# WeeFav/Visual-Odometry-GPU

Measured on AMD Instinct MI355X. Metric: ORB detect+describe frames/sec (1241x376, 8 lvls), higher is better.
Workload: dtype u8; 1 GPU; KITTI-shaped 1241x376 u8, 8 levels s=1.2, 1000 features, FAST-9 t=20, NMS 3x3, Harris top-N, blur5 all levels, BRIEF-256; batch=1024 frames/step/GPU resident in HBM (stream A); distinct_resident_batches=2, fast_early_exit=True, pyramid_blur_fused=True, pyramid_top_rows_first=True, pipelined_batches=True

## Files before the change

### visual-odometry-gpu_amd/csrc/orbx_api.cpp

```cpp
#include <algorithm>
#include <array>
#include <cmath>
#include <cstdlib>
#include <cstring>
#include <new>

#include "orbx_host.h"

using namespace orbx_host;

namespace {
thread_local std::string g_create_error;
}

namespace orbx_host {

int fail(orbx_ctx* c, int status, const std::string& msg) {
  if (c)
    c->err = msg;
  else
    g_create_error = msg;
  return status;
}

// ... 169 lines not shown
}

int pyr_group_env() {
  static const int v = env_int("ORBX_PYR_GROUP", 32);
  return v;
}

int top_rows_env() {
  static const int v = std::max(env_int("ORBX_TOP_ROWS", 2), 0);
  return v;
}

int fast_impl_env() { return env_int("ORBX_FAST_IMPL", 4) == 3 ? 3 : 4; }

void first_split_env(orbx_ctx* c) {
  const char* e = getenv("ORBX_TOP_ROWS");
  e = e ? std::strchr(e, ':') : nullptr;
  while (e && *e == ':') {
    e++;
    if (!std::strncmp(e, "equal", 5)) {
      c->first_split = false;
    } else if (!std::strncmp(e, "trace", 5)) {
      c->split_trace = true;
    } else {
      for (int l = 0; l < ORBX_MAX_LEVELS; l++) {
        char* end = nullptr;
        const long v = std::strtol(e, &end, 10);
        if (end == e) break;
        c->cut_force[l] = (int)std::min<long>(std::max<long>(v, 0), 0xffff);
        e = end;
        if (*e != ',') break;
        e++;
      }
    }
    e = std::strchr(e, ':');
  }
}
int fast_unit_rows_max(const orbx_ctx* c) {
  return c->fast_impl == 4 ? ORBX_FAST_UNIT_ROWS_MAX : orbx_fast3_tile_h(c->p.nms_window / 2);
}

void make_taps(OrbxPlan& plan, std::vector<OrbxResizeTap>* taps) {
  taps->assign(taps_count(plan), OrbxResizeTap{0, 0, 0});
  for (int l = 1; l < plan.nlevels; l++) {
    const OrbxLevel& L = plan.L[l];
    const double scale_x = 1. / ((double)L.w / plan.w0), scale_y = 1. / ((double)L.h / plan.h0);
// ... 167 lines not shown
    int first[ORBX_MAX_LEVELS][2] = {};
    bool any = false;
    for (int l = 0; l < plan.nlevels; l++) {
      int a = c->cut_force[l] > 0 ? c->cut_force[l] : c->cut_pref[l];
      if (a <= 0 || c->bm_fast.tiles_y[l] < 2) continue;
      const int depth = 2 * c->bm_fast.tile_h[l], umax = fast_unit_rows_max(c);
      if (c->cut_force[l] > 0)
        a = std::max(std::max(1, depth - umax), std::min(a, std::min(umax, std::min(depth, plan.L[l].h) - 1)));
      first[l][0] = a;
      first[l][1] = depth - a;
      any = true;
    }
    if (any)
      (void)make_bandmap(plan, c->p.nms_window / 2, &c->bm_fast, &why, c->fast_impl == 4,
                         c->prefs_applied ? c->tile_h_pref : nullptr, first);
  }
  const bool grouped = pyr_group_env() > 0;
  const int top = top_rows_env();
  std::vector<OrbxTileDesc> t;
  blur_tiles_for_impl(c->blur_impl, plan, &t);
  if ((st = upload_tiles(c, T_BLUR, t, "blur tile table exceeds pool")) != ORBX_OK) return st;
  build_pyrblur_tiles(plan, ORBX_PYRBLUR_RH, &t, grouped);
  if ((st = upload_tiles(c, T_PYRBLUR, t, "strip table exceeds pool")) != ORBX_OK) return st;
  build_pyrblur_tiles(plan, ORBX_PYRBLUR_RH, &t, grouped, 1, &c->bm_fast, top);
  if ((st = upload_tiles(c, T_PYRBLUR_TOP, t, "strip table exceeds pool")) != ORBX_OK) return st;
  build_pyrblur_tiles(plan, ORBX_PYRBLUR_RH, &t, grouped, 2, &c->bm_fast, top);
  if ((st = upload_tiles(c, T_PYRBLUR_REST, t, "strip table exceeds pool")) != ORBX_OK) return st;
  c->top_levels = OrbxTopLevels{};
  for (int l = 0; l < plan.nlevels; l++)
    if (pyrblur_first_pass_rows(plan, c->bm_fast, l, top) < plan.L[l].h) {
      const int i = c->top_levels.n++;
      c->top_levels.stat_index[i] = l * ORBX_MAX_BANDS;
      c->top_levels.rows[i] = std::min(top, c->bm_fast.tiles_y[l]);
      c->top_levels.cap[i] = plan.L[l].cap;
    }
  build_pyrblur_tiles(plan, ORBX_PYRBLUR_RH_SMALL, &t);
  if ((st = upload_tiles(c, T_PYRBLUR_SMALL, t, "strip table exceeds pool")) != ORBX_OK) return st;
  build_frame_tiles(plan, ORBX_PYR2_TW, ORBX_PYR2_TH, true, &t);
  if ((st = upload_tiles(c, T_PYR2, t, "pyramid tile table exceeds pool")) != ORBX_OK) return st;
  build_fast_tiles(plan, c->bm_fast, 0, 1, &t);
  if ((st = upload_tiles(c, T_FAST, t, "FAST tile table exceeds pool")) != ORBX_OK) return st;
  c->plan_serial++;
  c->plan_w = w;
  c->plan_h = h;
  return ORBX_OK;
}

hipError_t launch_pyramid_auto(orbx_ctx* c, hipStream_t s, int n, const uint8_t* d_in, int in_stride,
                               size_t in_frame_stride) {
// ... 94 lines not shown
    const int dflt = orbx_fast3_tile_h(c->p.nms_window / 2), lh = c->plan.L[l].h;
    const int bal = (lh + (lh + dflt - 1) / dflt - 1) / ((lh + dflt - 1) / dflt);
    int hh = (rows + top - 1) / top;
    if (c->fast_impl == 4) {
      const int over = (hh + 2 * (c->p.nms_window / 2)) % 7;
      if ((over == 1 || over == 2) && top * (hh - over) >= (int)need + 3) hh -= over;
    }
    if (hh >= bal || lh <= top * hh) hh = 0;
    const int eff = hh ? hh : bal, cur = c->bm_fast.tile_h[l], asked = c->tile_h_pref[l] ? c->tile_h_pref[l] : bal;
    want[l] = ((eff > cur && (int)need > top * cur) || eff + 2 < std::min(cur, asked)) ? hh : c->tile_h_pref[l];
    if (eff > cur && (int)need > top * cur) grow = true;
    else if (eff + 2 < std::min(cur, asked)) change = true;
  }
  const bool heights_change = grow || change;
  const bool split = c->first_split && top == 2 && c->fast_impl == 4;
  const int R = c->p.nms_window / 2;
  int cut_want[ORBX_MAX_LEVELS] = {};
  bool cut_change = false;
  for (int l = 0; l < nl; l++) {
    uint32_t hist[ORBX_FILL_BUCKETS];
    uint64_t total = 0;
    for (int b = 0; b < ORBX_FILL_BUCKETS; b++) {
      hist[b] = c->fill_cur[l][b] + c->fill_prev[l][b];
      c->fill_prev[l][b] = c->fill_cur[l][b];
      c->fill_cur[l][b] = 0;
      total += hist[b];
    }
    if (!split || c->cut_force[l] > 0 || c->bm_fast.tiles_y[l] < 2) continue;
    const int dflt = orbx_fast3_tile_h(R), lh = c->plan.L[l].h;
    const int bal = (lh + (lh + dflt - 1) / dflt - 1) / ((lh + dflt - 1) / dflt);
    const int th_after = heights_change ? (want[l] ? want[l] : bal) : c->bm_fast.tile_h[l];
    const int depth = 2 * th_after;
    const int in_force = !heights_change && c->bm_fast.first_h[l][0] > 0 ? c->bm_fast.first_h[l][0] : 0;
    int cost_new = 0;
    const int cut_new = total && lh > depth ? choose_first_cut(hist, depth, R, ORBX_FAST_UNIT_ROWS_MAX, &cost_new) : 0;
    const int cost_now = first_pass_cost_milli(hist, depth, in_force ? in_force : depth / 2, R);
    if (!total || lh <= depth) cost_new = cost_now;
    const bool pays = cost_now - cost_new >= 1000, stopped = in_force && !cut_new && cost_now > cost_new;
    cut_want[l] = heights_change || pays || stopped ? cut_new : c->cut_pref[l];
    if (cut_want[l] != in_force && (pays || stopped)) cut_change = true;
    if (c->split_trace) {
      fprintf(stderr, "orbx split: batch %lld level %d need %u depth %d cut %d -> %d (%d -> %d milli-groups) fill rows:",
              c->batch_serial, l, c->need_prev[l], depth, in_force, cut_want[l], cost_now, cost_new);
      for (int b = 0; b < ORBX_FILL_BUCKETS; b++)
        if (hist[b]) fprintf(stderr, " %d:%u", ORBX_FILL_BUCKET_ROWS * (b + 1), hist[b]);
      fprintf(stderr, "\n");
// ... 77 lines not shown
                                 (int32_t*)(B.d + o.counts), (orbx_keypoint*)(B.d + o.lkp),
                                 (float*)(B.d + o.resp), (int32_t*)(B.d + o.level),
                                 (orbx_keypoint*)(B.d + o.kp), (uint32_t*)(B.d + o.kp16),
                                 (float*)(B.d + o.angle),
                                 (orbx_descriptor*)(B.d + o.desc), two_pass ? c->d_feedback : nullptr,
                                 two_pass ? const_cast<uint32_t*>(c->h_feedback) : nullptr, &hr));
  HIPCHK(c, mark(7, false));
  return ORBX_OK;
}

void drop_graph(orbx_ctx* c, int i) {
  if (c->g_exec[i]) (void)hipGraphExecDestroy(c->g_exec[i]);
  c->g_exec[i] = nullptr;
}

int run_batch(orbx_ctx* c, const uint8_t* d_frames, int n, int w, int h, int row_stride, size_t frame_stride,
              hipStream_t s, bool may_pipeline = false) {
  if (w != c->learn_w || h != c->learn_h) {
    c->learn_w = w;
    c->learn_h = h;
    for (int l = 0; l < ORBX_MAX_LEVELS; l++) c->need_cur[l] = c->need_prev[l] = 0, c->tile_h_pref[l] = c->cut_pref[l] = 0;
    std::memset(c->fill_cur, 0, sizeof(c->fill_cur));
    std::memset(c->fill_prev, 0, sizeof(c->fill_prev));
    for (int i = 2; i < ORBX_FEEDBACK_WORDS; i++) c->h_feedback[i] = 0;
    c->need_batches = 0;
    c->need_window = 2;
    c->retiles = 0;
  } else if (w == c->plan_w && h == c->plan_h) {
    bool any_pref = false;
    for (int l = 0; l < ORBX_MAX_LEVELS; l++) any_pref |= c->tile_h_pref[l] != 0 || c->cut_pref[l] != 0 || c->cut_force[l] != 0;
    if (adapt_tile_rows(c) || (any_pref && tile_prefs_apply(c) != c->prefs_applied)) c->plan_w = 0;
  }
  const bool lanes = may_pipeline && c->pipelined && s == c->stream && w == c->plan_w && h == c->plan_h;
  c->lane = lanes ? c->next_lane : 0;
  Lane& L = c->lanes[c->lane];
  if (lanes) {
    s = L.stream;
  } else {
    if (c->lanes[1].stream) HIPCHK(c, lanes_sync(c));
    if (c->last_stream && c->last_stream != s) HIPCHK(c, hipStreamSynchronize(c->last_stream));
  }
  int st = set_plan(c, w, h);
  if (st != ORBX_OK) return st;
  top_rows_update(c);
  const int blk = (c->blk + 1) % orbx_ctx::kBlocks;
  Block& B = c->blocks[blk];
// ... 443 lines not shown
  *total = (long long)c->bm_fast.band_begin[c->bm_fast.nbands] * n;
  *worked = fast_early_on(c) ? w : *total;
  return ORBX_OK;
}

int orbx_pyramid_pixel_counts(orbx_ctx* c, long long* produced, long long* total) {
  DeviceGuard _dg(c);
  if (!c || !produced || !total) return ORBX_ERR_INVALID_ARG;
  if (c->plan_w == 0 || last_block(c).n < 1) return fail(c, ORBX_ERR_INVALID_ARG, "run a batch first");
  const int n = last_block(c).n, top = top_rows_env();
  long long per_frame = 0;
  for (int l = 0; l < c->plan.nlevels; l++) per_frame += (long long)c->plan.L[l].w * c->plan.L[l].h;
  *total = per_frame * n;
  *produced = *total;
  if (!c->last_two_pass) return ORBX_OK;
  std::vector<unsigned long long> h((size_t)n * ORBX_FAST_STAT_WORDS);
  HIPCHK(c, hipStreamSynchronize(c->last_stream));
  HIPCHK(c, hipMemcpy(h.data(), cur_lane(c).d_row_stat, h.size() * 8, hipMemcpyDeviceToHost));
  long long done = 0;
  for (int f = 0; f < n; f++)
    for (int l = 0; l < c->plan.nlevels; l++) {
      const OrbxLevel& L = c->plan.L[l];
      const int first = pyrblur_first_pass_rows(c->plan, c->bm_fast, l, top);
      long long surv = 0;
      for (int b = 0; b < std::min(top, c->bm_fast.tiles_y[l]); b++)
        surv += (long long)(uint32_t)h[(size_t)f * ORBX_FAST_STAT_WORDS + (size_t)l * ORBX_MAX_BANDS + b];
      done += (long long)L.w * (first < L.h && surv >= L.cap ? first : L.h);
    }
  *produced = done;
  return ORBX_OK;
}

int orbx_enable_stage_timing(orbx_ctx* c, int enable) {
  DeviceGuard _dg(c);
  if (!c) return ORBX_ERR_INVALID_ARG;
  c->timing = enable < 0 || enable > 2 ? 1 : enable;
  return ORBX_OK;
}

int orbx_stage_times_history(orbx_ctx* c, int back, float* ms) {
  DeviceGuard _dg(c);
  if (!c || !ms) return ORBX_ERR_INVALID_ARG;
  if (back < 0 || back >= ORBX_EVENT_SETS || back >= c->ev_calls)
    return fail(c, ORBX_ERR_INVALID_ARG, "no timed batched call that far back");
  const long long call = c->ev_calls - 1 - back;
  const TimingSet& ts = c->evr[call % ORBX_EVENT_SETS];
  const hipEvent_t* evs = ts.ev;
  const int mode = ts.mode;
  std::memset(ms, 0, sizeof(float) * ORBX_NUM_STAGE_TIMES);
  if (mode == 1) {
// ... 257 lines not shown
```

### visual-odometry-gpu_amd/csrc/orbx_host.h

```cpp
#pragma once
#include <hip/hip_runtime.h>

#include <cmath>
#include <cstring>
#include <initializer_list>
#include <string>
#include <vector>

#include "orbx_internal.h"
#include "orbx_layout.h"

namespace orbx_host {

using namespace orbx_geom;
using namespace orbx_layout;

struct DevBuf {
  void* p = nullptr;
  size_t bytes = 0;
};
template <class T>
T* at(const DevBuf& b, size_t off) { return reinterpret_cast<T*>(static_cast<uint8_t*>(b.p) + off); }
inline void free_bufs(std::initializer_list<DevBuf*> bufs) {
  for (DevBuf* b : bufs)
// ... 274 lines not shown
  orbx_host::Landmarks lm;
  orbx_host::TracksPose tp;
  orbx_host::WindowPoses wp;
  orbx_host::StreamStitch st;

  int timing = 0;
  int fast_early = 1;
  int blur_impl = 2;
  int fast_impl = 4;
  int fuse = 1;
  int top_mode = 2;
  bool top_on = true;
  int top_single_batches = 0;
  uint32_t* d_feedback = nullptr;
  volatile uint32_t* h_feedback = nullptr;
  uint32_t feedback_seen[2] = {0, 0};
  uint32_t need_cur[ORBX_MAX_LEVELS] = {}, need_prev[ORBX_MAX_LEVELS] = {};
  int tile_h_pref[ORBX_MAX_LEVELS] = {};
  int need_batches = 0, need_window = 2, retiles = 0, learn_w = 0, learn_h = 0;
  bool prefs_applied = false;
  uint32_t fill_cur[ORBX_MAX_LEVELS][ORBX_FILL_BUCKETS] = {}, fill_prev[ORBX_MAX_LEVELS][ORBX_FILL_BUCKETS] = {};
  int cut_pref[ORBX_MAX_LEVELS] = {}, cut_force[ORBX_MAX_LEVELS] = {};
  bool first_split = true, split_trace = false;
  orbx_host::TimingSet evr[ORBX_EVENT_SETS];
  long long ev_calls = 0;
  hipEvent_t ev[2] = {};
};

namespace orbx_host {

struct DeviceGuard {
  int prev = -1;
  bool switched = false;
  explicit DeviceGuard(const orbx_ctx* c) {
    if (!c) return;
    enter(c->device);
  }
  explicit DeviceGuard(int dev) { enter(dev); }
  void enter(int dev) {
    if (hipGetDevice(&prev) == hipSuccess && prev != dev) switched = hipSetDevice(dev) == hipSuccess;
  }
  ~DeviceGuard() {
    if (switched) (void)hipSetDevice(prev);
  }
  DeviceGuard(const DeviceGuard&) = delete;
  DeviceGuard& operator=(const DeviceGuard&) = delete;
// ... 71 lines not shown
```

### visual-odometry-gpu_amd/csrc/orbx_kernels.hip

```cpp
#include <hip/hip_runtime.h>

#include <cstdlib>

#include "orbx_internal.h"
#include "orbx_math.h"
#include "orbx_wave.h"

__constant__ __attribute__((aligned(16))) int8_t c_pattern[1024] = {
#include "pattern_31.inc"
};


typedef uint16_t __attribute__((aligned(1))) u16_unaligned;

__device__ __forceinline__ void decode_tile(const OrbxTileMap& tm, int nlevels, int& l, int& tx, int& ty) {
  const int t = blockIdx.x;
  l = 0;
#pragma unroll 1
  for (int i = 1; i < nlevels; i++)
    if (t >= tm.begin[i]) l = i;
  const int local = t - tm.begin[l];
  ty = local / tm.tiles_x[l];
  tx = local - ty * tm.tiles_x[l];
}
// ... 1027 lines not shown
    }
    desc_out[k] = __ballot(bit);
  }
}



#define DESC_NLD ((DESC_ROWS * (DESC_PITCH / 4) + 63) / 64)

struct DescClip {
  int rlo, rhi, clo, chi;
};
__device__ __forceinline__ DescClip desc_clip(const DescJob& jb) {
  const int py0 = jb.y - DESC_R, ax0 = (jb.x - DESC_R) & ~3;
  return {max(-py0, 0), min(jb.h - 1 - py0, DESC_ROWS - 1), max(-ax0, 0), min(jb.pitch - 4 - ax0, DESC_PITCH - 4)};
}
enum { DESC_INSIDE = 0, DESC_TOP = 1, DESC_CLIPPED = 2 };
__device__ __forceinline__ int desc_kind(const DescJob& jb) {
  const int py0 = jb.y - DESC_R, ax0 = (jb.x - DESC_R) & ~3;
  const bool below = py0 + DESC_ROWS <= jb.h, cols = ax0 >= 0 && ax0 + DESC_PITCH <= jb.pitch;
  return below && cols ? (py0 >= 0 ? DESC_INSIDE : DESC_TOP) : DESC_CLIPPED;
}

template <int KIND>
__device__ __forceinline__ void desc_fetch_border(const DescJob& jb, uint32_t base, const int (&rowk)[DESC_NLD],
                                                  const int (&c3)[3], uint32_t (&regs)[DESC_NLD]) {
  const DescClip cl = desc_clip(jb);
  int cb[3];
#pragma unroll
  for (int m = 0; m < 3; m++) cb[m] = KIND == DESC_TOP ? 4 * c3[m] : min(max(4 * c3[m], cl.clo), cl.chi);
#pragma unroll
  for (int k = 0; k < DESC_NLD; k++) {
    const int r = KIND == DESC_TOP ? max(rowk[k], cl.rlo) : min(max(rowk[k], cl.rlo), cl.rhi);
    regs[k] = *reinterpret_cast<const uint32_t*>(
        jb.img + (base + (__umul24((uint32_t)r, (uint32_t)jb.pitch) + (uint32_t)cb[k % 3])));
  }
}

struct DescLds2 {
  uint32_t patch[DESC_ROWS * DESC_PITCH / 4];
  uint16_t hs[DESC_ROWS * DESC_HP];
};

template <class L>
__device__ __forceinline__ void desc_store_patch(L& lds, int lane, const uint32_t (&regs)[DESC_NLD]) {
#pragma unroll
  for (int k = 0; k < DESC_NLD; k++)
    if (lane + 64 * k < DESC_ROWS * (DESC_PITCH / 4)) lds.patch[lane + 64 * k] = regs[k];
}

// ... 65 lines not shown
        acc.x = pk_sub(pk_add(acc.x, nw.x), od.x);
        acc.y = pk_sub(pk_add(acc.y, nw.y), od.y);
        q[(i - 1) % 5] = nw;
        bp[i * (DESC_HP / 4)] = acc;
      }
    }
  }
  wave_lds_sync();
}

__device__ __forceinline__ float lround_f(float v) {
  const float t = __builtin_truncf(v);
  const float fr = __fsub_rn(v, t);
  return __fadd_rn(t, __builtin_truncf(__fadd_rn(fr, fr)));
}

typedef float f2_t __attribute__((ext_vector_type(2)));
typedef int i2_t __attribute__((ext_vector_type(2)));
__device__ __forceinline__ i2_t lround_small2(f2_t v) {
  const f2_t h = {0.5f - 0x1p-25f, 0.5f - 0x1p-25f};
  return __builtin_convertvector(v + __builtin_elementwise_copysign(h, v), i2_t);
}

template <int DESC_KPW, int DESC_NW, int DESC_OCC>
__global__ __launch_bounds__(64 * DESC_NW, DESC_OCC) void k_describe2(OrbxPlan plan, const uint8_t* __restrict__ pyr, int patch_size,
                                                   const int32_t* __restrict__ sel_count,
                                                   const orbx_keypoint* __restrict__ sel_lkp,
                                                   const float* __restrict__ sel_resp,
                                                   int32_t* __restrict__ out_count,
                                                   orbx_keypoint* __restrict__ out_lkp,
                                                   float* __restrict__ out_resp,
                                                   int32_t* __restrict__ out_level,
                                                   orbx_keypoint* __restrict__ out_kp,
                                                   uint32_t* __restrict__ out_kp16,
                                                   float* __restrict__ out_angle,
                                                   orbx_descriptor* __restrict__ out_desc,
                                                   const uint32_t* __restrict__ feedback, uint32_t* __restrict__ feedback_host,
                                                   OrbxHostRecord host) {
  constexpr int DESC_KPB = DESC_NW * DESC_KPW;
  static_assert(2 * DESC_KPB <= 64 * DESC_NW, "trig: two threads per keypoint");
  __shared__ __attribute__((aligned(16))) DescLds2 s_lds[DESC_NW];
  __shared__ int s_m[DESC_KPB][2];
  __shared__ float s_cs[DESC_KPB][2];
  __shared__ uint2 s_mw[4 * (DESC_PITCH / 4)];
  __shared__ __attribute__((aligned(16))) uint32_t s_rec_kp[DESC_KPB], s_rec_angle[DESC_KPB], s_rec_desc[DESC_KPB][8];
  const int f = blockIdx.x, grp = blockIdx.y, tid = threadIdx.x, lane = tid & 63;
  const int wave = __builtin_amdgcn_readfirstlane(tid >> 6);
  static_assert(ORBX_MAX_LEVELS <= 64, "one lane per level");
  const int lvl_cnt = lane < plan.nlevels ? sel_count[f * plan.nlevels + lane] : 0;
  const int lvl_end = wave_scan_incl(lvl_cnt);
  const int count = __builtin_amdgcn_readlane(lvl_end, 63);
  if (grp == 0 && tid == 0) {
    out_count[f] = count;
    if (host.counts) host.counts[f] = count;
  }
  if (feedback_host && grp == 0 && f == 0)
    for (int i = tid; i < ORBX_FEEDBACK_WORDS; i += (int)blockDim.x) feedback_host[i] = feedback[i];
  const int slot0 = grp * DESC_KPB;
  if (slot0 >= count) return;
  DescLds2& lds = s_lds[wave];
  const int pr = patch_size / 2;
  if (tid < 4 * (DESC_PITCH / 4)) {
    const int off = tid / (DESC_PITCH / 4), c = tid - off * (DESC_PITCH / 4);
    uint32_t xw = 0, on = 0;
#pragma unroll
    for (int b = 0; b < 4; b++) {
      const int t = 4 * c + b - off - (DESC_R - pr);
      if (t >= 0 && t <= 2 * pr) {
        xw |= (uint32_t)t << (8 * b);
        on |= 1u << (8 * b);
      }
    }
    s_mw[tid] = make_uint2(xw, on);
  }
  int rowk[DESC_NLD], c3[3];
  uint32_t rin = 0;
  {
    int row = lane / (DESC_PITCH / 4), c = lane - row * (DESC_PITCH / 4);
#pragma unroll
    for (int k = 0; k < DESC_NLD; k++) {
      rowk[k] = min(row, DESC_ROWS - 1);
      __builtin_assume(rowk[k] >= 0 && rowk[k] < DESC_ROWS);
      if (k < 3) c3[k] = c;
      if (lane + 64 * k < DESC_ROWS * (DESC_PITCH / 4) && row >= DESC_R - pr && row <= DESC_R + pr) rin |= 1u << k;
      row += 5;
      c += 4;
      if (c >= DESC_PITCH / 4) {
        c -= DESC_PITCH / 4;
        row += 1;
      }
    }
  }
  __syncthreads();
  const size_t fo = (size_t)f * plan.out_cap;

  const int nk = min(DESC_KPW, max(0, count - (slot0 + wave * DESC_KPW)));
  DescJob jobs[DESC_KPW];
  float scale[DESC_KPW];
  uint32_t regs[DESC_KPW][DESC_NLD];
  int offs[DESC_KPW];
#pragma unroll
  for (int j = 0; j < DESC_KPW; j++) {
    const int slot = min(slot0 + wave * DESC_KPW + j, count - 1);
    const int level = __popcll(__ballot(lvl_end <= slot));
    const int lvl_begin = __builtin_amdgcn_readlane(lvl_end - lvl_cnt, level);
    const size_t src = fo + plan.L[level].out_off + (slot - lvl_begin);
    const orbx_keypoint kp = sel_lkp[src];
    jobs[j] = desc_job(plan, pyr, f, kp, level);
    scale[j] = plan.L[level].scale;
    if (j < nk && lane == 0) {
      out_lkp[fo + slot] = kp;
      out_resp[fo + slot] = sel_resp[src];
      out_level[fo + slot] = level;
    }
  }
#pragma unroll
  for (int j = 0; j < DESC_KPW; j++) {
    const DescJob& jb = jobs[j];
    const int py0 = jb.y - DESC_R, ax0 = (jb.x - DESC_R) & ~3;
    offs[j] = jb.x - DESC_R - ax0;
    const uint32_t base = (uint32_t)(py0 * jb.pitch + ax0);
    const int kind = desc_kind(jb);
    if (kind == DESC_INSIDE) {
#pragma unroll
      for (int k = 0; k < DESC_NLD; k++) {
        regs[j][k] = 0;
        if (lane + 64 * k < DESC_ROWS * (DESC_PITCH / 4))
          regs[j][k] = *reinterpret_cast<const uint32_t*>(jb.img + (base + (__umul24((uint32_t)rowk[k], (uint32_t)jb.pitch) + 4u * (uint32_t)c3[k % 3])));
      }
    } else if (kind == DESC_TOP) {
      desc_fetch_border<DESC_TOP>(jb, base, rowk, c3, regs[j]);
    } else {
      desc_fetch_border<DESC_CLIPPED>(jb, base, rowk, c3, regs[j]);
    }
  }

  int pm[2][DESC_KPW];
#pragma unroll
  for (int j = 0; j < DESC_KPW; j++) {
    const DescJob& jb = jobs[j];
    const int off = offs[j];
    pm[0][j] = pm[1][j] = 0;
    if (j < nk && !(jb.x - pr < 0 || jb.x + pr >= jb.w || jb.y - pr < 0 || jb.y + pr >= jb.h)) {
      uint2 mw[3];
#pragma unroll
      for (int m = 0; m < 3; m++) mw[m] = s_mw[off * (DESC_PITCH / 4) + c3[m]];
      uint32_t X = 0, S = 0, M = 0;
#pragma unroll
      for (int k = 0; k < DESC_NLD; k++) {
        const uint32_t z = regs[j][k] & (uint32_t)(-(int32_t)((rin >> k) & 1u));
        X = __builtin_amdgcn_udot4(z, mw[k % 3].x, X, false);
        const uint32_t rs = __builtin_amdgcn_udot4(z, mw[k % 3].y, 0u, false);
        S += rs;
        M += __umul24((uint32_t)rowk[k], rs);
      }
      pm[0][j] = (int)X - __mul24(pr, (int)S);
      pm[1][j] = (int)M - __mul24(DESC_R, (int)S);
    }
  }
  if constexpr (DESC_KPW == 4) {
    int u[2];
#pragma unroll
    for (int i = 0; i < 2; i++) {
      const auto h0 = __builtin_amdgcn_permlane32_swap(pm[i][0], pm[i][1], false, false);
      const auto h1 = __builtin_amdgcn_permlane32_swap(pm[i][2], pm[i][3], false, false);
      const auto r = __builtin_amdgcn_permlane16_swap(h0[0] + h0[1], h1[0] + h1[1], false, false);
      u[i] = row_sum16(r[0] + r[1]);
    }
    if ((lane & 15) == 0) {
      const int q = wave * DESC_KPW + (((lane >> 4) & 1) << 1 | (lane >> 5));
      s_m[q][0] = u[0];
      s_m[q][1] = u[1];
    }
  } else {
#pragma unroll
    for (int j = 0; j < DESC_KPW; j++) {
      const int m10 = wave_sum(pm[0][j]), m01 = wave_sum(pm[1][j]);
// ... 267 lines not shown
  const bool spread = mode == ORBX_SELECT_HARRIS &&
                      (lvl_slots(plan, plan.nlevels) > LVL_MAX_SLOTS ||
                       (force >= 0 ? force != 0 : maxcap > LVL_THREADS));
  if (!spread)
    return orbx_launch_level_select(s, plan, n_frames, mode, d_mask, d_pyr, d_gauss, window, k, d_sel_lkp,
                                    d_sel_resp, d_sel_count, d_need);
  hipLaunchKernelGGL(k_lvl_compact, dim3(plan.nlevels, n_frames), dim3(256), 0, s, plan, d_mask, d_cand, d_ncand, d_need);
  hipLaunchKernelGGL(k_lvl_harris, dim3((maxcap + 255) / 256, plan.nlevels, n_frames), dim3(256), 0, s, plan, d_pyr,
                     d_gauss, window, k, d_cand, d_ncand, d_cresp);
  const size_t lds = (size_t)((maxcap + 7) & ~7) * 8;
  hipLaunchKernelGGL(k_lvl_rank, dim3((maxcap + RANK_SLICE - 1) / RANK_SLICE, plan.nlevels, n_frames), dim3(256), lds,
                     s, plan, d_cand, d_ncand, d_cresp, d_sel_lkp, d_sel_resp, d_sel_count);
  return ORBX_LAUNCH_CHECK();
}

hipError_t orbx_launch_describe(hipStream_t s, const OrbxPlan& plan, int n_frames, const uint8_t* d_pyr,
                                int patch_size, const int32_t* d_sel_count, const orbx_keypoint* d_sel_lkp,
                                const float* d_sel_resp, int32_t* d_out_count, orbx_keypoint* d_out_lkp,
                                float* d_out_resp, int32_t* d_out_level, orbx_keypoint* d_out_kp, uint32_t* d_out_kp16,
                                float* d_out_angle, orbx_descriptor* d_out_desc, const uint32_t* d_feedback,
                                uint32_t* h_feedback, const OrbxHostRecord* host_record) {
  const OrbxHostRecord host = host_record ? *host_record : OrbxHostRecord{};
  if (plan.out_cap <= 0) return hipSuccess;
  if ((long long)plan.out_cap * n_frames <= 8192) {
    dim3 grid(n_frames, (plan.out_cap + 3) / 4);
    hipLaunchKernelGGL((k_describe2<1, 4, 1>), grid, dim3(256), 0, s, plan, d_pyr, patch_size, d_sel_count, d_sel_lkp,
                       d_sel_resp, d_out_count, d_out_lkp, d_out_resp, d_out_level, d_out_kp, d_out_kp16, d_out_angle, d_out_desc, d_feedback,
                       h_feedback, host);
  } else {
    dim3 grid(n_frames, (plan.out_cap + 15) / 16);
    hipLaunchKernelGGL((k_describe2<4, 4, 6>), grid, dim3(256), 0, s, plan, d_pyr, patch_size, d_sel_count, d_sel_lkp,
                       d_sel_resp, d_out_count, d_out_lkp, d_out_resp, d_out_level, d_out_kp, d_out_kp16, d_out_angle, d_out_desc, d_feedback,
                       h_feedback, host);
  }
  return ORBX_LAUNCH_CHECK();
}

hipError_t orbx_launch_describe_flat(hipStream_t s, const uint8_t* d_img, int w, int h, int pitch,
                                     const orbx_keypoint* d_kps, int nkp, int patch_size, int use_given_angles,
                                     int do_brief, float* d_angles, orbx_descriptor* d_desc) {
  if (nkp <= 0) return hipSuccess;
  hipLaunchKernelGGL(k_describe_flat, dim3((nkp + 3) / 4), dim3(256), 0, s, d_img, w, h, pitch, d_kps, nkp,
                     patch_size, use_given_angles, do_brief, d_angles, d_desc);
  return ORBX_LAUNCH_CHECK();
}

hipError_t orbx_launch_harris_flat(hipStream_t s, const uint8_t* d_img, int w, int h, int pitch,
                                   const orbx_keypoint* d_kps, int nkp, const float* d_gauss, int K, float kk,
                                   float* d_resp) {
  if (nkp <= 0) return hipSuccess;
  hipLaunchKernelGGL(k_harris2_flat, dim3((nkp + 31) / 32), dim3(256), 0, s, d_img, w, h, pitch, d_kps, nkp,
                     d_gauss, K, kk, d_resp);
  return ORBX_LAUNCH_CHECK();
}
// ... 36 lines not shown
```

### visual-odometry-gpu_amd/csrc/orbx_plan.h

```cpp
#pragma once
#include <stddef.h>
#include <stdint.h>

#include <algorithm>
#include <cmath>
#include <cstring>
#include <string>
#include <vector>

#include "../../include/orbx.h"

struct OrbxLevel {
  int32_t w, h, pitch;
  int32_t img_off;
  int32_t mask_wpr;
  int32_t mask_off;
  int32_t cap;
  int32_t quota;
  int32_t cand_off;
  int32_t xtab_off;
  int32_t ytab_off;
  float scale;
  int32_t out_off;
  int32_t win8;
// ... 279 lines not shown
        d.w = L.w;
        d.h = L.h;
        d.pitch = L.pitch;
        d.img_off = (uint64_t)L.img_off;
        if (d.ty < L.h) {
          if (out) out->push_back(d);
          cnt++;
        }
      }
  }
  return cnt;
}

inline size_t blur_tiles_for_impl(int impl, const OrbxPlan& plan, std::vector<OrbxTileDesc>* out) {
  return impl == 3 ? build_blur4_tiles(plan, out) : build_blur_tiles(plan, out);
}

inline int pyrblur_first_pass_rows(const OrbxPlan& plan, const OrbxBandMap& bm, int l, int top_rows) {
  if (top_rows <= 0 || bm.tiles_y[l] <= top_rows) return plan.L[l].h;
  int y0, rows;
  fast_band_rows(bm, l, top_rows - 1, &y0, &rows);
  return std::min(plan.L[l].h, y0 + rows + ORBX_TOP_MARGIN);
}
inline size_t build_pyrblur_tiles(const OrbxPlan& plan, int max_rows, std::vector<OrbxTileDesc>* out,
                                  bool heavy_first = false, int part = 0, const OrbxBandMap* bm = nullptr,
                                  int top_rows = 0) {
  size_t cnt = 0;
  if (out) out->clear();
  bool have_reporter = false;
  for (int l = 0; l < plan.nlevels; l++) {
    const OrbxLevel& L = plan.L[l];
    const int dw = (L.w + 3) / 4;
    const int ntx = dw <= 64 ? 1 : (dw - 2 + 61) / 62;
    const int split = part == 0 ? L.h : pyrblur_first_pass_rows(plan, *bm, l, top_rows);
    const int r0 = part == 2 ? split : 0, r1 = part == 1 ? split : L.h;
    if (r1 <= r0) continue;
    const int nb = (r1 - r0 + max_rows - 1) / max_rows, rows = (r1 - r0 + nb - 1) / nb;
    for (int b = 0; b < nb; b++)
      for (int tx = 0; tx < ntx; tx++) {
        OrbxTileDesc d{};
        d.l = l;
        d.tx = tx;
        d.ty = r0 + b * rows;
        d.f = std::min(rows, r1 - d.ty);
        d.w = L.w;
        d.h = L.h;
        d.pitch = L.pitch;
        d.u0 = L.xtab_off;
        d.u1 = L.ytab_off;
        d.u2 = L.win8;
        d.pad = (uint32_t)ntx;
        d.img_off = (uint64_t)L.img_off;
        if (part == 2) {
          d.stat_index = (uint32_t)(l * ORBX_MAX_BANDS);
          d.mask_off = ((uint64_t)(uint32_t)std::min(top_rows, bm->tiles_y[l]) << 32) | (uint32_t)L.cap;
          if (b == 0 && tx == 0 && !have_reporter) {
            d.mask_off |= 1ull << 62;
            have_reporter = true;
          }
        }
        if (d.f > 0) {
          if (out) out->push_back(d);
          cnt++;
        }
      }
  }
  if (heavy_first && out) {
    auto cost = [](const OrbxTileDesc& d) { return (d.f + 4) * (d.l == 0 ? 35 : d.u2 == 1 ? 80 : 90); };
    std::stable_sort(out->begin(), out->end(),
                     [&](const OrbxTileDesc& a, const OrbxTileDesc& b) { return cost(a) > cost(b); });
  }
  return cnt;
}

inline int build_plan(const orbx_params& p, int w0, int h0, OrbxPlan* plan, std::string* why, int fast_impl = 3) {
  std::memset(plan, 0, sizeof(*plan));
  plan->nlevels = p.nlevels;
  plan->w0 = w0;
  plan->h0 = h0;
  size_t img_off = 0, mask_off = 0;
  int cand_off = 0, out_cap = 0, xt = 0;
  for (int l = 0; l < p.nlevels; l++) {
    OrbxLevel& L = plan->L[l];
    level_size(w0, h0, p.scale_factor, l, &L.w, &L.h);
    if (L.w < 8 || L.h < 8) {
      *why = "pyramid level " + std::to_string(l) + " is smaller than 8x8 (" + std::to_string(L.w) + "x" +
             std::to_string(L.h) + ")";
      return ORBX_ERR_UNSUPPORTED;
    }
    L.pitch = align_up(L.w, 64);
    L.img_off = (int32_t)img_off;
// ... 30 lines not shown
      *why = "pyramid frame exceeds 2 GiB";
      return ORBX_ERR_UNSUPPORTED;
    }
  }
  plan->frame_bytes = (int32_t)img_off;
  plan->mask_words = (int32_t)mask_off;
  plan->cand_total = std::max(cand_off, (out_cap + 15) & ~15);
  plan->out_cap = (out_cap + 15) & ~15;
  return ORBX_OK;
}

inline size_t taps_count(const OrbxPlan& plan) {
  size_t total = 0;
  for (int l = 1; l < plan.nlevels; l++) total += (size_t)align_up(plan.L[l].w, 4) + align_up(plan.L[l].h, 4);
  return total ? total : 1;
}

struct OrbxTableCapacity {
  size_t fast;
  size_t frame;
  size_t small;
  size_t taps;
};
inline size_t fast_tiles_upper_bound(const OrbxPlan& M, int nms_radius, bool strips) {
  size_t cap = 0;
  for (int l = 0; l < M.nlevels; l++) {
    const int rows = std::min(ORBX_MAX_BANDS, (M.L[l].h + ORBX_MIN_TILE_H - 1) / ORBX_MIN_TILE_H);
    cap += (size_t)fast_tiles_x(M.L[l].w, nms_radius, strips) * (size_t)rows;
  }
  return cap;
}
inline int table_capacity(const orbx_params& p, const OrbxPlan& M, int fast_impl, int blur_impl, OrbxTableCapacity* cap,
                          std::string* why) {
  OrbxBandMap bm;
  const int st = make_bandmap(M, p.nms_window / 2, &bm, why, fast_impl == 4, nullptr);
  if (st != ORBX_OK) return st;
  cap->fast = fast_tiles_upper_bound(M, p.nms_window / 2, fast_impl == 4);
  const size_t t1 = blur_tiles_for_impl(blur_impl, M, nullptr);
  const size_t t2 = build_frame_tiles(M, ORBX_PYR2_TW, ORBX_PYR2_TH, true, nullptr);
  const size_t t3 = build_pyrblur_tiles(M, ORBX_PYRBLUR_RH, nullptr);
  cap->frame = std::max(std::max(t1, t2), t3) + 256;
  cap->small = build_pyrblur_tiles(M, ORBX_PYRBLUR_RH_SMALL, nullptr) + 64;
  cap->taps = taps_count(M) + 16;
  return ORBX_OK;
}

#define ORBX_FILL_BUCKETS 32
#define ORBX_FILL_BUCKET_ROWS 4
inline int fill_bucket(int fill_row) { return std::min(std::max(fill_row - 1, 0) / ORBX_FILL_BUCKET_ROWS, ORBX_FILL_BUCKETS - 1); }
inline uint32_t fill_exits(const uint32_t* hist, int cut) {
  uint32_t n = 0;
  for (int b = 0; b < ORBX_FILL_BUCKETS - 1 && ORBX_FILL_BUCKET_ROWS * (b + 1) <= cut; b++) n += hist[b];
  return n;
}
#define ORBX_FAST4_UNIT_SETUP_MILLI 1200
#define ORBX_FAST4_UNIT_EXIT_MILLI 280
struct OrbxUnitCost {
  int setup_milli, exit_milli;
};
inline int fast4_unit_cost_milli(int rows, int nms_radius, const OrbxUnitCost& uc) {
  return uc.setup_milli + 1000 * ((rows + 2 * nms_radius + 6) / 7);
}
inline int first_pass_cost_milli(const uint32_t* hist, int depth, int cut, int nms_radius,
                                 const OrbxUnitCost& uc = OrbxUnitCost{ORBX_FAST4_UNIT_SETUP_MILLI, ORBX_FAST4_UNIT_EXIT_MILLI}) {
// ... 3 lines not shown
  const uint64_t second = (on * (uint64_t)fast4_unit_cost_milli(depth - cut, nms_radius, uc) + out * (uint64_t)uc.exit_milli) /
                          (total ? total : 1);
  return fast4_unit_cost_milli(cut, nms_radius, uc) + (int)second;
}
inline int choose_first_cut(const uint32_t* hist, int depth, int nms_radius, int unit_max, int* cost_milli,
                            const OrbxUnitCost& uc = OrbxUnitCost{ORBX_FAST4_UNIT_SETUP_MILLI, ORBX_FAST4_UNIT_EXIT_MILLI}) {
  uint64_t total = 0;
  for (int b = 0; b < ORBX_FILL_BUCKETS; b++) total += hist[b];
  int best = 0, best_cost = first_pass_cost_milli(hist, depth, depth / 2, nms_radius, uc);
  if (total)
    for (int cut = 7 - (2 * nms_radius) % 7; cut < depth; cut += 7) {
      if (cut > unit_max || depth - cut > unit_max || cut == depth / 2) continue;
      if (fill_exits(hist, cut) == 0) continue;
      const int c = first_pass_cost_milli(hist, depth, cut, nms_radius, uc);
      if (c < best_cost) {
        best = cut;
        best_cost = c;
      }
    }
  if (cost_milli) *cost_milli = best_cost;
  return best;
}

}
```

Measured before the change: 682,800 frames/s.

## Split pyramid blur first pass with an early band and specialize describe for radius 15

New measurement: 695,200 frames/s (median of 6 runs). +1.8%, better.

```diff
diff --git a/visual-odometry-gpu_amd/csrc/orbx_api.cpp b/visual-odometry-gpu_amd/csrc/orbx_api.cpp
--- a/visual-odometry-gpu_amd/csrc/orbx_api.cpp
+++ b/visual-odometry-gpu_amd/csrc/orbx_api.cpp
@@ -215,6 +215,8 @@
       c->first_split = false;
     } else if (!std::strncmp(e, "trace", 5)) {
       c->split_trace = true;
+    } else if (!std::strncmp(e, "late", 4)) {
+      c->early_band = false;
     } else {
       for (int l = 0; l < ORBX_MAX_LEVELS; l++) {
         char* end = nullptr;
@@ -428,9 +430,23 @@
   if ((st = upload_tiles(c, T_BLUR, t, "blur tile table exceeds pool")) != ORBX_OK) return st;
   build_pyrblur_tiles(plan, ORBX_PYRBLUR_RH, &t, grouped);
   if ((st = upload_tiles(c, T_PYRBLUR, t, "strip table exceeds pool")) != ORBX_OK) return st;
-  build_pyrblur_tiles(plan, ORBX_PYRBLUR_RH, &t, grouped, 1, &c->bm_fast, top);
+  for (int l = 0; l < ORBX_MAX_LEVELS; l++) c->early_rows[l] = 0;
+  for (int l = 0; l < plan.nlevels; l++) {
+    const int late = pyrblur_first_pass_rows(plan, c->bm_fast, l, top);
+    const int P = c->early_band ? pyrblur_early_rows(plan, c->bm_fast, l, top, c->p.nms_window / 2) : late;
+    const bool forced = c->cut_force[l] > 0;
+    const bool pays = P < late && (forced ? late - P >= ORBX_PYRBLUR_EARLY_MIN_ROWS
+                                          : early_band_pays(c->fill_last[l], c->bm_fast.first_h[l][0], late - P,
+                                                            pyrblur_row_cost(l, plan.L[l].win8)));
+    c->early_rows[l] = pays ? P : late;
+    if (c->split_trace && c->bm_fast.first_h[l][0] > 0)
+      fprintf(stderr, "orbx early band: level %d cut %d first pass ended at %d, now ends at %d, band %d rows: %s\n", l,
+              c->bm_fast.first_h[l][0], late, c->early_rows[l], late - P,
+              pays ? (forced ? "split (forced cut)" : "split") : !c->early_band ? "late" : "kept");
+  }
+  build_pyrblur_tiles(plan, ORBX_PYRBLUR_RH, &t, grouped, 1, &c->bm_fast, top, c->early_rows);
   if ((st = upload_tiles(c, T_PYRBLUR_TOP, t, "strip table exceeds pool")) != ORBX_OK) return st;
-  build_pyrblur_tiles(plan, ORBX_PYRBLUR_RH, &t, grouped, 2, &c->bm_fast, top);
+  build_pyrblur_tiles(plan, ORBX_PYRBLUR_RH, &t, grouped, 2, &c->bm_fast, top, c->early_rows);
   if ((st = upload_tiles(c, T_PYRBLUR_REST, t, "strip table exceeds pool")) != ORBX_OK) return st;
   c->top_levels = OrbxTopLevels{};
   for (int l = 0; l < plan.nlevels; l++)
@@ -571,6 +587,7 @@
     uint64_t total = 0;
     for (int b = 0; b < ORBX_FILL_BUCKETS; b++) {
       hist[b] = c->fill_cur[l][b] + c->fill_prev[l][b];
+      c->fill_last[l][b] = hist[b];
       c->fill_prev[l][b] = c->fill_cur[l][b];
       c->fill_cur[l][b] = 0;
       total += hist[b];
@@ -694,6 +711,7 @@
     for (int l = 0; l < ORBX_MAX_LEVELS; l++) c->need_cur[l] = c->need_prev[l] = 0, c->tile_h_pref[l] = c->cut_pref[l] = 0;
     std::memset(c->fill_cur, 0, sizeof(c->fill_cur));
     std::memset(c->fill_prev, 0, sizeof(c->fill_prev));
+    std::memset(c->fill_last, 0, sizeof(c->fill_last));
     for (int i = 2; i < ORBX_FEEDBACK_WORDS; i++) c->h_feedback[i] = 0;
     c->need_batches = 0;
     c->need_window = 2;
@@ -1183,10 +1201,14 @@
     for (int l = 0; l < c->plan.nlevels; l++) {
       const OrbxLevel& L = c->plan.L[l];
       const int first = pyrblur_first_pass_rows(c->plan, c->bm_fast, l, top);
-      long long surv = 0;
-      for (int b = 0; b < std::min(top, c->bm_fast.tiles_y[l]); b++)
+      long long surv = 0, surv0 = 0;
+      for (int b = 0; b < std::min(top, c->bm_fast.tiles_y[l]); b++) {
         surv += (long long)(uint32_t)h[(size_t)f * ORBX_FAST_STAT_WORDS + (size_t)l * ORBX_MAX_BANDS + b];
-      done += (long long)L.w * (first < L.h && surv >= L.cap ? first : L.h);
+        if (b == 0) surv0 = surv;
+      }
+      const int early = c->early_rows[l] > 0 && c->early_rows[l] < first ? c->early_rows[l] : first;
+      const int band = surv0 >= L.cap ? 0 : first - early;
+      done += (long long)L.w * (first < L.h && surv >= L.cap ? early + band : L.h);
     }
   *produced = done;
   return ORBX_OK;
diff --git a/visual-odometry-gpu_amd/csrc/orbx_host.h b/visual-odometry-gpu_amd/csrc/orbx_host.h
--- a/visual-odometry-gpu_amd/csrc/orbx_host.h
+++ b/visual-odometry-gpu_amd/csrc/orbx_host.h
@@ -320,6 +320,9 @@
   uint32_t fill_cur[ORBX_MAX_LEVELS][ORBX_FILL_BUCKETS] = {}, fill_prev[ORBX_MAX_LEVELS][ORBX_FILL_BUCKETS] = {};
   int cut_pref[ORBX_MAX_LEVELS] = {}, cut_force[ORBX_MAX_LEVELS] = {};
   bool first_split = true, split_trace = false;
+  uint32_t fill_last[ORBX_MAX_LEVELS][ORBX_FILL_BUCKETS] = {};
+  int early_rows[ORBX_MAX_LEVELS] = {};
+  bool early_band = true;
   orbx_host::TimingSet evr[ORBX_EVENT_SETS];
   long long ev_calls = 0;
   hipEvent_t ev[2] = {};
diff --git a/visual-odometry-gpu_amd/csrc/orbx_kernels.hip b/visual-odometry-gpu_amd/csrc/orbx_kernels.hip
--- a/visual-odometry-gpu_amd/csrc/orbx_kernels.hip
+++ b/visual-odometry-gpu_amd/csrc/orbx_kernels.hip
@@ -1073,10 +1073,12 @@
   return below && cols ? (py0 >= 0 ? DESC_INSIDE : DESC_TOP) : DESC_CLIPPED;
 }
 
-template <int KIND>
+template <int KIND, uint32_t RB>
 __device__ __forceinline__ void desc_fetch_border(const DescJob& jb, uint32_t base, const int (&rowk)[DESC_NLD],
                                                   const int (&c3)[3], uint32_t (&regs)[DESC_NLD]) {
-  const DescClip cl = desc_clip(jb);
+  DescClip cl = desc_clip(jb);
+  cl.rlo |= (int)RB;
+  cl.rhi |= (int)RB;
   int cb[3];
 #pragma unroll
   for (int m = 0; m < 3; m++) cb[m] = KIND == DESC_TOP ? 4 * c3[m] : min(max(4 * c3[m], cl.clo), cl.chi);
@@ -1188,7 +1190,35 @@
   return __builtin_convertvector(v + __builtin_elementwise_copysign(h, v), i2_t);
 }
 
-template <int DESC_KPW, int DESC_NW, int DESC_OCC>
+template <int ORAD>
+struct DescWindow {
+  static constexpr int RD = DESC_PITCH / 4;
+  static constexpr int lo = (DESC_R - ORAD) * RD, hi = (DESC_R + ORAD + 1) * RD;
+  static constexpr int lane_lo(int k) { return lo - 64 * k < 0 ? 0 : lo - 64 * k > 64 ? 64 : lo - 64 * k; }
+  static constexpr int lane_hi(int k) { return hi - 64 * k < 0 ? 0 : hi - 64 * k > 64 ? 64 : hi - 64 * k; }
+  static constexpr bool none(int k) { return lane_lo(k) >= lane_hi(k); }
+  static constexpr bool all(int k) { return lane_lo(k) == 0 && lane_hi(k) == 64; }
+  static constexpr int count() {
+    int n = 0;
+    for (int k = 0; k < DESC_NLD; k++) n += !none(k);
+    return n;
+  }
+};
+static_assert(DescWindow<15>::none(7) && DescWindow<15>::count() == 7, "radius 15: dwords 0 ... 6");
+static_assert(DescWindow<15>::all(1) && DescWindow<15>::all(2) && DescWindow<15>::all(3) && DescWindow<15>::all(4) &&
+                  DescWindow<15>::all(5),
+              "radius 15: dwords 1 ... 5 take no mask");
+static_assert(DescWindow<15>::lane_lo(0) == (DESC_R - 15) * (DESC_PITCH / 4) && DescWindow<15>::lane_hi(0) == 64,
+              "radius 15: dword 0 from the first dword of the window's first row");
+static_assert(DescWindow<15>::lane_lo(6) == 0 &&
+                  DescWindow<15>::lane_hi(6) == (DESC_R + 15 + 1) * (DESC_PITCH / 4) - 6 * 64,
+              "radius 15: dword 6 up to the last dword of the window's last row");
+#define DESC_WS 19
+static_assert(DESC_NLD * 1020 * (DESC_ROWS - 1) < (1 << DESC_WS), "M fits below S in W");
+static_assert((long long)DESC_NLD * 1020 < (1ll << (32 - DESC_WS)), "W fits 32 bits");
+static_assert(DESC_ROWS <= (1 << DESC_WS) && DESC_WS < 23, "24-bit factors");
+
+template <int DESC_KPW, int DESC_NW, int DESC_OCC, int ORAD>
 __global__ __launch_bounds__(64 * DESC_NW, DESC_OCC) void k_describe2(OrbxPlan plan, const uint8_t* __restrict__ pyr, int patch_size,
                                                    const int32_t* __restrict__ sel_count,
                                                    const orbx_keypoint* __restrict__ sel_lkp,
@@ -1225,7 +1255,7 @@
   const int slot0 = grp * DESC_KPB;
   if (slot0 >= count) return;
   DescLds2& lds = s_lds[wave];
-  const int pr = patch_size / 2;
+  const int pr = ORAD != 0 ? ORAD : patch_size / 2;
   if (tid < 4 * (DESC_PITCH / 4)) {
     const int off = tid / (DESC_PITCH / 4), c = tid - off * (DESC_PITCH / 4);
     uint32_t xw = 0, on = 0;
@@ -1239,14 +1269,15 @@
     }
     s_mw[tid] = make_uint2(xw, on);
   }
+  constexpr uint32_t RB = ORAD != 0 ? 1u << DESC_WS : 0u;
   int rowk[DESC_NLD], c3[3];
   uint32_t rin = 0;
   {
     int row = lane / (DESC_PITCH / 4), c = lane - row * (DESC_PITCH / 4);
 #pragma unroll
     for (int k = 0; k < DESC_NLD; k++) {
-      rowk[k] = min(row, DESC_ROWS - 1);
-      __builtin_assume(rowk[k] >= 0 && rowk[k] < DESC_ROWS);
+      rowk[k] = min(row, DESC_ROWS - 1) | (int)RB;
+      __builtin_assume(rowk[k] >= (int)RB && rowk[k] < (int)RB + DESC_ROWS);
       if (k < 3) c3[k] = c;
       if (lane + 64 * k < DESC_ROWS * (DESC_PITCH / 4) && row >= DESC_R - pr && row <= DESC_R + pr) rin |= 1u << k;
       row += 5;
@@ -1285,7 +1316,7 @@
     const DescJob& jb = jobs[j];
     const int py0 = jb.y - DESC_R, ax0 = (jb.x - DESC_R) & ~3;
     offs[j] = jb.x - DESC_R - ax0;
-    const uint32_t base = (uint32_t)(py0 * jb.pitch + ax0);
+    const uint32_t base = (uint32_t)(py0 * jb.pitch + ax0) - RB * (uint32_t)jb.pitch;
     const int kind = desc_kind(jb);
     if (kind == DESC_INSIDE) {
 #pragma unroll
@@ -1295,9 +1326,9 @@
           regs[j][k] = *reinterpret_cast<const uint32_t*>(jb.img + (base + (__umul24((uint32_t)rowk[k], (uint32_t)jb.pitch) + 4u * (uint32_t)c3[k % 3])));
       }
     } else if (kind == DESC_TOP) {
-      desc_fetch_border<DESC_TOP>(jb, base, rowk, c3, regs[j]);
+      desc_fetch_border<DESC_TOP, RB>(jb, base, rowk, c3, regs[j]);
     } else {
-      desc_fetch_border<DESC_CLIPPED>(jb, base, rowk, c3, regs[j]);
+      desc_fetch_border<DESC_CLIPPED, RB>(jb, base, rowk, c3, regs[j]);
     }
   }
 
@@ -1312,13 +1343,28 @@
 #pragma unroll
       for (int m = 0; m < 3; m++) mw[m] = s_mw[off * (DESC_PITCH / 4) + c3[m]];
       uint32_t X = 0, S = 0, M = 0;
-#pragma unroll
-      for (int k = 0; k < DESC_NLD; k++) {
-        const uint32_t z = regs[j][k] & (uint32_t)(-(int32_t)((rin >> k) & 1u));
-        X = __builtin_amdgcn_udot4(z, mw[k % 3].x, X, false);
-        const uint32_t rs = __builtin_amdgcn_udot4(z, mw[k % 3].y, 0u, false);
-        S += rs;
-        M += __umul24((uint32_t)rowk[k], rs);
+      if constexpr (ORAD != 0) {
+        using Wn = DescWindow<ORAD>;
+        uint32_t W = 0;
+#pragma unroll
+        for (int k = 0; k < DESC_NLD; k++) {
+          if (Wn::none(k)) continue;
+          const uint32_t z = Wn::all(k) || (lane >= Wn::lane_lo(k) && lane < Wn::lane_hi(k)) ? regs[j][k] : 0u;
+          X = __builtin_amdgcn_udot4(z, mw[k % 3].x, X, false);
+          const uint32_t rs = __builtin_amdgcn_udot4(z, mw[k % 3].y, 0u, false);
+          W += __umul24((uint32_t)rowk[k], rs);
+        }
+        S = W >> DESC_WS;
+        M = W & ((1u << DESC_WS) - 1);
+      } else {
+#pragma unroll
+        for (int k = 0; k < DESC_NLD; k++) {
+          const uint32_t z = regs[j][k] & (uint32_t)(-(int32_t)((rin >> k) & 1u));
+          X = __builtin_amdgcn_udot4(z, mw[k % 3].x, X, false);
+          const uint32_t rs = __builtin_amdgcn_udot4(z, mw[k % 3].y, 0u, false);
+          S += rs;
+          M += __umul24((uint32_t)rowk[k], rs);
+        }
       }
       pm[0][j] = (int)X - __mul24(pr, (int)S);
       pm[1][j] = (int)M - __mul24(DESC_R, (int)S);
@@ -1632,14 +1678,15 @@
                                 uint32_t* h_feedback, const OrbxHostRecord* host_record) {
   const OrbxHostRecord host = host_record ? *host_record : OrbxHostRecord{};
   if (plan.out_cap <= 0) return hipSuccess;
+  const bool win31 = patch_size == 31;
   if ((long long)plan.out_cap * n_frames <= 8192) {
     dim3 grid(n_frames, (plan.out_cap + 3) / 4);
-    hipLaunchKernelGGL((k_describe2<1, 4, 1>), grid, dim3(256), 0, s, plan, d_pyr, patch_size, d_sel_count, d_sel_lkp,
+    hipLaunchKernelGGL((win31 ? k_describe2<1, 4, 1, 15> : k_describe2<1, 4, 1, 0>), grid, dim3(256), 0, s, plan, d_pyr, patch_size, d_sel_count, d_sel_lkp,
                        d_sel_resp, d_out_count, d_out_lkp, d_out_resp, d_out_level, d_out_kp, d_out_kp16, d_out_angle, d_out_desc, d_feedback,
                        h_feedback, host);
   } else {
     dim3 grid(n_frames, (plan.out_cap + 15) / 16);
-    hipLaunchKernelGGL((k_describe2<4, 4, 6>), grid, dim3(256), 0, s, plan, d_pyr, patch_size, d_sel_count, d_sel_lkp,
+    hipLaunchKernelGGL((win31 ? k_describe2<4, 4, 6, 15> : k_describe2<4, 4, 6, 0>), grid, dim3(256), 0, s, plan, d_pyr, patch_size, d_sel_count, d_sel_lkp,
                        d_sel_resp, d_out_count, d_out_lkp, d_out_resp, d_out_level, d_out_kp, d_out_kp16, d_out_angle, d_out_desc, d_feedback,
                        h_feedback, host);
   }
diff --git a/visual-odometry-gpu_amd/csrc/orbx_plan.h b/visual-odometry-gpu_amd/csrc/orbx_plan.h
--- a/visual-odometry-gpu_amd/csrc/orbx_plan.h
+++ b/visual-odometry-gpu_amd/csrc/orbx_plan.h
@@ -325,51 +325,67 @@
   fast_band_rows(bm, l, top_rows - 1, &y0, &rows);
   return std::min(plan.L[l].h, y0 + rows + ORBX_TOP_MARGIN);
 }
+inline int pyrblur_early_rows(const OrbxPlan& plan, const OrbxBandMap& bm, int l, int top_rows, int nms_radius) {
+  const int late = pyrblur_first_pass_rows(plan, bm, l, top_rows);
+  if (top_rows != 2 || bm.tiles_y[l] <= top_rows || bm.first_h[l][0] <= 0 || late >= plan.L[l].h) return late;
+  const int h0 = bm.first_h[l][0], D = h0 + bm.first_h[l][1];
+  return std::min(late, std::max(h0 + ORBX_TOP_MARGIN, D + nms_radius + 3));
+}
+inline int pyrblur_strips_x(int w) {
+  const int dw = (w + 3) / 4;
+  return dw <= 64 ? 1 : (dw - 2 + 61) / 62;
+}
+inline int pyrblur_row_cost(int l, int win8) { return l == 0 ? 35 : win8 == 1 ? 80 : 90; }
+#define ORBX_PYRBLUR_WARMUP_ROWS 4
 inline size_t build_pyrblur_tiles(const OrbxPlan& plan, int max_rows, std::vector<OrbxTileDesc>* out,
                                   bool heavy_first = false, int part = 0, const OrbxBandMap* bm = nullptr,
-                                  int top_rows = 0) {
+                                  int top_rows = 0, const int* early_rows = nullptr) {
   size_t cnt = 0;
   if (out) out->clear();
   bool have_reporter = false;
   for (int l = 0; l < plan.nlevels; l++) {
     const OrbxLevel& L = plan.L[l];
-    const int dw = (L.w + 3) / 4;
-    const int ntx = dw <= 64 ? 1 : (dw - 2 + 61) / 62;
+    const int ntx = pyrblur_strips_x(L.w);
     const int split = part == 0 ? L.h : pyrblur_first_pass_rows(plan, *bm, l, top_rows);
-    const int r0 = part == 2 ? split : 0, r1 = part == 1 ? split : L.h;
-    if (r1 <= r0) continue;
-    const int nb = (r1 - r0 + max_rows - 1) / max_rows, rows = (r1 - r0 + nb - 1) / nb;
-    for (int b = 0; b < nb; b++)
-      for (int tx = 0; tx < ntx; tx++) {
-        OrbxTileDesc d{};
-        d.l = l;
-        d.tx = tx;
-        d.ty = r0 + b * rows;
-        d.f = std::min(rows, r1 - d.ty);
-        d.w = L.w;
-        d.h = L.h;
-        d.pitch = L.pitch;
-        d.u0 = L.xtab_off;
-        d.u1 = L.ytab_off;
-        d.u2 = L.win8;
-        d.pad = (uint32_t)ntx;
-        d.img_off = (uint64_t)L.img_off;
-        if (part == 2) {
-          d.stat_index = (uint32_t)(l * ORBX_MAX_BANDS);
-          d.mask_off = ((uint64_t)(uint32_t)std::min(top_rows, bm->tiles_y[l]) << 32) | (uint32_t)L.cap;
-          if (b == 0 && tx == 0 && !have_reporter) {
-            d.mask_off |= 1ull << 62;
-            have_reporter = true;
+    const int early = part != 0 && early_rows && early_rows[l] > 0 && early_rows[l] < split ? early_rows[l] : split;
+    const int seg[2][3] = {{part == 2 ? early : 0, part == 1 ? early : part == 2 ? split : L.h, 1},
+                           {split, part == 2 ? L.h : split, std::min(top_rows, bm ? bm->tiles_y[l] : 0)}};
+    for (int s = 0; s < 2; s++) {
+      const int r0 = seg[s][0], r1 = seg[s][1];
+      if (r1 <= r0) continue;
+      const int nb = (r1 - r0 + max_rows - 1) / max_rows, rows = (r1 - r0 + nb - 1) / nb;
+      for (int b = 0; b < nb; b++)
+        for (int tx = 0; tx < ntx; tx++) {
+          OrbxTileDesc d{};
+          d.l = l;
+          d.tx = tx;
+          d.ty = r0 + b * rows;
+          d.f = std::min(rows, r1 - d.ty);
+          d.w = L.w;
+          d.h = L.h;
+          d.pitch = L.pitch;
+          d.u0 = L.xtab_off;
+          d.u1 = L.ytab_off;
+          d.u2 = L.win8;
+          d.pad = (uint32_t)ntx;
+          d.img_off = (uint64_t)L.img_off;
+          if (part == 2) {
+            d.stat_index = (uint32_t)(l * ORBX_MAX_BANDS);
+            d.mask_off = ((uint64_t)(uint32_t)seg[s][2] << 32) | (uint32_t)L.cap;
+            if (s == 1 && b == 0 && tx == 0 && !have_reporter) {
+              d.mask_off |= 1ull << 62;
+              have_reporter = true;
+            }
+          }
+          if (d.f > 0) {
+            if (out) out->push_back(d);
+            cnt++;
           }
         }
-        if (d.f > 0) {
-          if (out) out->push_back(d);
-          cnt++;
-        }
-      }
+    }
   }
   if (heavy_first && out) {
-    auto cost = [](const OrbxTileDesc& d) { return (d.f + 4) * (d.l == 0 ? 35 : d.u2 == 1 ? 80 : 90); };
+    auto cost = [](const OrbxTileDesc& d) { return (d.f + ORBX_PYRBLUR_WARMUP_ROWS) * pyrblur_row_cost(d.l, d.u2); };
     std::stable_sort(out->begin(), out->end(),
                      [&](const OrbxTileDesc& a, const OrbxTileDesc& b) { return cost(a) > cost(b); });
   }
@@ -446,6 +462,12 @@
   size_t small;
   size_t taps;
 };
+static_assert(ORBX_TOP_MARGIN <= ORBX_PYRBLUR_RH, "an early band is one band");
+inline size_t pyrblur_early_strips_bound(const OrbxPlan& M) {
+  size_t n = 0;
+  for (int l = 0; l < M.nlevels; l++) n += (size_t)pyrblur_strips_x(M.L[l].w);
+  return n;
+}
 inline size_t fast_tiles_upper_bound(const OrbxPlan& M, int nms_radius, bool strips) {
   size_t cap = 0;
   for (int l = 0; l < M.nlevels; l++) {
@@ -463,7 +485,7 @@
   const size_t t1 = blur_tiles_for_impl(blur_impl, M, nullptr);
   const size_t t2 = build_frame_tiles(M, ORBX_PYR2_TW, ORBX_PYR2_TH, true, nullptr);
   const size_t t3 = build_pyrblur_tiles(M, ORBX_PYRBLUR_RH, nullptr);
-  cap->frame = std::max(std::max(t1, t2), t3) + 256;
+  cap->frame = std::max(std::max(t1, t2), t3) + 256 + pyrblur_early_strips_bound(M);
   cap->small = build_pyrblur_tiles(M, ORBX_PYRBLUR_RH_SMALL, nullptr) + 64;
   cap->taps = taps_count(M) + 16;
   return ORBX_OK;
@@ -513,4 +535,15 @@
   return best;
 }
 
-}
+#define ORBX_PYRBLUR_SKIP_EXIT 100
+#define ORBX_PYRBLUR_EARLY_MIN_ROWS 3
+inline bool early_band_pays(const uint32_t* hist, int h0, int rows, int row_cost, int exit_cost = ORBX_PYRBLUR_SKIP_EXIT) {
+  uint64_t total = 0;
+  for (int b = 0; b < ORBX_FILL_BUCKETS; b++) total += hist[b];
+  if (!total || rows < ORBX_PYRBLUR_EARLY_MIN_ROWS) return false;
+  const uint64_t out = fill_exits(hist, h0), stay = total - out;
+  return out * (uint64_t)rows * (uint64_t)row_cost >
+         stay * (uint64_t)(ORBX_PYRBLUR_WARMUP_ROWS * row_cost) + out * (uint64_t)exit_cost;
+}
+
+}
```
